# ardaduz/deep-video-mvs

Hardware: AMD Instinct MI355X
Metric: depth frames/sec/GPU @ 320x256x64 planes (fusionnet); rel-L1 vs ref (higher is better)
Workload: dtype f32

## Files before the change

deep-video-mvs_amd/csrc/direct_conv.hip:

```cpp
#include <stdlib.h>

#include "dvmvs_device.h"

namespace dvmvs {

typedef float float4v __attribute__((ext_vector_type(4)));

struct DirectConvArgs {
  const float* x;
  const float* packed;
  const float* bias;
  float* dst;
  float* dst_nhwc;
  long long x_batch_stride, dst_batch_stride;
  int B, C_in, C_out, H, W, OH, OW;
  int act;
  int n_groups;
  int packed_groups;
  int n_chunks;
  int tiles_x;
  int vec4;
};

#ifdef DVMVS_SWEEP_TRACE
constexpr int kDcTraceWords = 8, kDcTraceWaves = 16384;
__device__ unsigned long long g_dc_trace[kDcTraceWaves * kDcTraceWords];
#define DC_TRACE(...) __VA_ARGS__
#define DC_NOW() __builtin_amdgcn_s_memrealtime()
#else
#define DC_TRACE(...)
#endif

constexpr int kDcGroupPad = 16;

__host__ __device__ constexpr int dc_round_to_residue(int v, int mod, int res) { return v + ((res - v) % mod + mod) % mod; }

template <int K_, int S_, int MW_, int MT_, int NT_, int PW_, int KS_, int G_>
struct DirectConvConfig {
  static constexpr int K = K_, S = S_, MW = MW_, MT = MT_, NTILE = NT_, PW = PW_, KS = KS_, G = G_;
  static constexpr int MH = 16 / MW;
  static constexpr int NWAVES = PW * KS, NT = 64 * NWAVES;
  static constexpr int CIC = 4 * KS * G;
  static constexpr int TILE_H = PW * MH, TILE_W = MW * MT;
  static constexpr int PH = (TILE_H - 1) * S + K, PWD = TILE_W * S + 8, PWD4 = PWD / 4;
  static constexpr int SHIFT = 4 - K / 2;
  static constexpr int RS = (MH == 1) ? PWD : dc_round_to_residue(PWD, 16, 8);
  static constexpr int CS = dc_round_to_residue(PH * RS, 64, 16);
  static constexpr int Q = (NTILE * K + 3) / 4;
  static constexpr int NS = G * K;
  static constexpr bool PRIVATE = PW == 1;
  static constexpr int STAGE_CH = PRIVATE ? 4 * G : CIC;
  static constexpr int STAGE_NT = PRIVATE ? 64 : NT;
  static constexpr int PATCH = STAGE_CH * PH * PWD4;
  static constexpr int XREGS = (PATCH + STAGE_NT - 1) / STAGE_NT;
  static constexpr int RED_FLOATS = (KS > 1) ? (KS / 2) * PW * MT * NTILE * 256 : 0;
  static constexpr int BUF = CIC * CS;
  static constexpr bool PREFETCH = XREGS <= 8;
  static constexpr bool DOUBLE = PREFETCH && sizeof(float) * 2 * BUF <= 150 * 1024;
  static constexpr bool WHOLE = DOUBLE && K == 3 && NS * Q <= 6;
  static constexpr int LDS_FLOATS = ((DOUBLE ? 2 : 1) * BUF > RED_FLOATS) ? (DOUBLE ? 2 : 1) * BUF : RED_FLOATS;
  static_assert((MW == 16 || MW == 8) && (TILE_W * S) % 4 == 0 && RS % 4 == 0 && CS % 4 == 0, "tile shape");
  static_assert(NWAVES == 8 && NS >= 2 && (kDcGroupPad % (KS * G)) == 0 && (KS & (KS - 1)) == 0, "workgroup shape");
  static_assert(sizeof(float) * LDS_FLOATS <= 160 * 1024, "LDS");
};

template <class Cfg>
__global__ __launch_bounds__(Cfg::NT) void direct_conv_kernel(DirectConvArgs a) {
  constexpr int K = Cfg::K, S = Cfg::S, MW = Cfg::MW, MT = Cfg::MT, NTILE = Cfg::NTILE, PW = Cfg::PW, KS = Cfg::KS, G = Cfg::G;
  constexpr int MH = Cfg::MH, CIC = Cfg::CIC, PH = Cfg::PH, PWD4 = Cfg::PWD4, RS = Cfg::RS, CS = Cfg::CS, Q = Cfg::Q, NS = Cfg::NS;
  constexpr int XREGS = Cfg::XREGS, PATCH = Cfg::PATCH, STAGE_NT = Cfg::STAGE_NT;
  constexpr bool PRIVATE = Cfg::PRIVATE;
  extern __shared__ __attribute__((aligned(16))) float s_x[];

  const int tid = threadIdx.x, lane = tid & 63, wave = __builtin_amdgcn_readfirstlane(tid >> 6);
  const int pw = wave % PW, ks = wave / PW;
  const int ty = blockIdx.x / a.tiles_x, tx = blockIdx.x - ty * a.tiles_x;
  const int cot = blockIdx.y, b = blockIdx.z;
  const int oy0 = ty * Cfg::TILE_H, ox0 = tx * Cfg::TILE_W;
  const int iy0 = oy0 * S - K / 2, ix0 = ox0 * S - 4;
  const int HW = a.H * a.W;
  DC_TRACE(const unsigned long long tr_start = DC_NOW(); unsigned long long tr_first = 0, tr_req = 0, tr_mfma = 0, tr_store = 0, tr_loop = 0, tr_red = 0, tr_a = 0, tr_b = 0, tr_c = 0;
           auto dump_trace = [&]() __attribute__((always_inline)) {
             const unsigned long long tr_end = DC_NOW();
             const size_t wv = (static_cast<size_t>(blockIdx.z * gridDim.y + blockIdx.y) * gridDim.x + blockIdx.x) * Cfg::NWAVES + (threadIdx.x >> 6);
             if ((threadIdx.x & 63) == 0 && wv < kDcTraceWaves) {
               unsigned long long* t = g_dc_trace + wv * kDcTraceWords;
               t[0] = tr_start; t[1] = tr_first; t[2] = tr_req; t[3] = tr_mfma; t[4] = tr_store; t[5] = tr_loop; t[6] = tr_red; t[7] = tr_end;
             }
           };)
  gcfloat_p xg = as_global(a.x) + static_cast<size_t>(b) * a.x_batch_stride;

  constexpr bool PREFETCH = Cfg::PREFETCH, DOUBLE = Cfg::DOUBLE, WHOLE = Cfg::WHOLE;
  constexpr int BUF = Cfg::BUF;
  const __amdgpu_buffer_rsrc_t x_resource =
      __builtin_amdgcn_make_buffer_rsrc((void*)xg, 0, static_cast<int>(sizeof(float) * static_cast<unsigned int>(a.C_in) * HW), 0x00020000);
  constexpr unsigned int kOutOfRange = 0x80000000u;
  const int stage_tid = PRIVATE ? lane : tid;
  const int stage_ch0 = PRIVATE ? ks * G * 4 : 0;
  auto element_offset = [&](int i) __attribute__((always_inline)) -> unsigned int {
    const int e = stage_tid + i * STAGE_NT;
    const int ch = e / (PH * PWD4), rem = e - ch * (PH * PWD4);
    const int row = rem / PWD4, col4 = rem - row * PWD4;
    const int iy = iy0 + row, ix = ix0 + 4 * col4;
    const bool in = e < PATCH && iy >= 0 && iy < a.H && ix >= 0 && ix < a.W;
    return in ? static_cast<unsigned int>(sizeof(float)) * static_cast<unsigned int>((stage_ch0 + ch) * HW + iy * a.W + ix) : kOutOfRange;
  };
  unsigned int x_offset[PREFETCH ? XREGS : 1];
  if (PREFETCH) {
#pragma unroll
    for (int i = 0; i < XREGS; ++i) x_offset[i] = element_offset(i);
  }
  auto load_element = [&](int chunk, int i) __attribute__((always_inline)) -> float4v {
    const unsigned int offset = PREFETCH ? x_offset[i] : element_offset(i);
    const bool live = chunk * CIC + stage_ch0 + (stage_tid + i * STAGE_NT) / (PH * PWD4) < a.C_in;
    return __builtin_bit_cast(float4v, __builtin_amdgcn_raw_buffer_load_b128(x_resource, static_cast<int>(live ? offset : kOutOfRange),
                                                                             static_cast<int>(sizeof(float) * static_cast<unsigned int>(chunk * CIC) * HW), 0));
  };
  auto store_element = [&](float* buffer, int i, float4v v) __attribute__((always_inline)) {
    const int e = stage_tid + i * STAGE_NT;
    const int ch = e / (PH * PWD4), rem = e - ch * (PH * PWD4);
    const int row = rem / PWD4, col4 = rem - row * PWD4;
    if (e < PATCH) *reinterpret_cast<float4v*>(buffer + (stage_ch0 + ch) * CS + row * RS + 4 * col4) = v;
  };
  float4v xr[PREFETCH ? XREGS : 1];
  auto load_patch = [&](int chunk) __attribute__((always_inline)) {
    if (PREFETCH) {
#pragma unroll
      for (int i = 0; i < XREGS; ++i) xr[i] = load_element(chunk, i);
    }
  };
  auto store_patch = [&](int chunk, float* buffer) __attribute__((always_inline)) {
    if (PREFETCH) {
#pragma unroll
      for (int i = 0; i < XREGS; ++i) store_element(buffer, i, xr[i]);
    } else {
#pragma unroll 1
      for (int i0 = 0; i0 < XREGS; i0 += 4) {
        float4v piece[4];
#pragma unroll
        for (int i = 0; i < 4; ++i) piece[i] = load_element(chunk, i0 + i);
#pragma unroll
        for (int i = 0; i < 4; ++i) store_element(buffer, i0 + i, piece[i]);
      }
    }
  };

  auto chunk_barrier = [&]() __attribute__((always_inline)) {
    if (PRIVATE) __builtin_amdgcn_wave_barrier();
    else __syncthreads();
  };

  const float4v DVMVS_GLOBAL* wq = reinterpret_cast<const float4v DVMVS_GLOBAL*>(as_global(a.packed)) +
                                   static_cast<size_t>(cot) * a.packed_groups * (K * Q * 64) + lane;
  auto load_weights = [&](float4v* w, int cg, int ky) __attribute__((always_inline)) {
    cg = min(cg, a.packed_groups - 1);
#pragma unroll
    for (int q = 0; q < Q; ++q) w[q] = wq[(static_cast<size_t>(cg) * K + ky) * (Q * 64) + q * 64];
  };

  const int m = lane & 15;
  const int a_base = ((lane >> 4) + ks * G * 4) * CS + ((pw * MH + m / MW) * S) * RS + (m % MW) * S + Cfg::SHIFT;

  float4v acc[MT][NTILE];
#pragma unroll
  for (int mt = 0; mt < MT; ++mt)
#pragma unroll
    for (int nt = 0; nt < NTILE; ++nt) acc[mt][nt] = float4v{0.0f, 0.0f, 0.0f, 0.0f};

  auto multiply_step = [&](const float* buffer, int gg, int ky, const float4v* w) __attribute__((always_inline)) {
#pragma unroll
    for (int kx = 0; kx < K; ++kx) {
#pragma unroll
      for (int mt = 0; mt < MT; ++mt) {
        const float av = buffer[a_base + gg * 4 * CS + ky * RS + kx + mt * MW * S];
#pragma unroll
        for (int nt = 0; nt < NTILE; ++nt) {
          const int j = kx * NTILE + nt;
          acc[mt][nt] = __builtin_amdgcn_mfma_f32_16x16x4f32(av, w[j / 4][j % 4], acc[mt][nt], 0, 0, 0);
        }
      }
    }
  };

  if (WHOLE) {
    float4v w_even[NS][Q], w_odd[NS][Q];
    auto whole_chunk = [&](int chunk, float4v(*w_use)[Q], float4v(*w_load)[Q]) __attribute__((always_inline)) {
      const int cg0 = (chunk * KS + ks) * G;
      const float* buffer = s_x + (chunk & 1) * BUF;
      DC_TRACE(tr_a = DC_NOW(); __builtin_amdgcn_sched_barrier(0);)
#pragma unroll
      for (int s = 0; s < NS; ++s) load_weights(w_load[s], ((chunk + 1) * KS + ks) * G + s / K, s % K);
      load_patch(chunk + 1);
      __builtin_amdgcn_sched_barrier(0);
      DC_TRACE(tr_b = DC_NOW(); __builtin_amdgcn_sched_barrier(0);)
#pragma unroll
      for (int s = 0; s < NS; ++s)
        if (cg0 + s / K < a.n_groups) multiply_step(buffer, s / K, s % K, w_use[s]);
      DC_TRACE(__builtin_amdgcn_sched_barrier(0); asm volatile("s_nop 0" ::"v"(acc[0][0]), "v"(acc[MT - 1][NTILE - 1])); tr_c = DC_NOW(); __builtin_amdgcn_sched_barrier(0);)
#pragma unroll
      for (int s = 0; s < NS; ++s) asm volatile("" ::"v"(w_load[s][Q - 1]), "v"(w_use[s][Q - 1]));
      store_patch(chunk + 1, s_x + ((chunk + 1) & 1) * BUF);
      chunk_barrier();
      DC_TRACE(tr_req += tr_b - tr_a; tr_mfma += tr_c - tr_b; tr_store += DC_NOW() - tr_c;)
    };
#pragma unroll
    for (int s = 0; s < NS; ++s) load_weights(w_even[s], ks * G + s / K, s % K);
    load_patch(0);
    store_patch(0, s_x);
    chunk_barrier();
    DC_TRACE(tr_first = DC_NOW();)
    for (int chunk = 0; chunk < a.n_chunks; chunk += 2) {
      whole_chunk(chunk, w_even, w_odd);
      if (chunk + 1 < a.n_chunks) whole_chunk(chunk + 1, w_odd, w_even);
    }
  } else {
    float4v wb[2][Q], w_next[Q];
    load_patch(0);
    load_weights(w_next, ks * G, 0);
    store_patch(0, s_x);
    chunk_barrier();
    DC_TRACE(tr_first = DC_NOW();)
    for (int chunk = 0; chunk < a.n_chunks; ++chunk) {
      const bool more = chunk + 1 < a.n_chunks;
      const int cg0 = (chunk * KS + ks) * G;
      const float* buffer = s_x + (DOUBLE ? (chunk & 1) * BUF : 0);
#pragma unroll
      for (int q = 0; q < Q; ++q) wb[0][q] = w_next[q];
      DC_TRACE(tr_a = tr_b = DC_NOW(); __builtin_amdgcn_sched_barrier(0);)
#pragma unroll
      for (int s = 0; s < NS; ++s) {
        if (s + 1 < NS) load_weights(wb[(s + 1) & 1], cg0 + (s + 1) / K, (s + 1) % K);
        if (s == NS - 2 && (more || DOUBLE)) load_patch(chunk + 1);
        if (s == NS - 1 && (more || DOUBLE)) load_weights(w_next, ((chunk + 1) * KS + ks) * G, 0);
        __builtin_amdgcn_sched_barrier(0);
        if (cg0 + s / K < a.n_groups) multiply_step(buffer, s / K, s % K, wb[s & 1]);
        asm volatile("" ::"v"(wb[s & 1][Q - 1]));
      }
      DC_TRACE(__builtin_amdgcn_sched_barrier(0); asm volatile("s_nop 0" ::"v"(acc[0][0]), "v"(acc[MT - 1][NTILE - 1])); tr_c = DC_NOW(); __builtin_amdgcn_sched_barrier(0);)
      if (DOUBLE) {
        store_patch(chunk + 1, s_x + ((chunk + 1) & 1) * BUF);
        chunk_barrier();
        DC_TRACE(tr_mfma += tr_c - tr_b; tr_store += DC_NOW() - tr_c;)
      } else {
        chunk_barrier();
        if (more) {
          store_patch(chunk + 1, s_x);
          chunk_barrier();
        }
      }
    }
  }

  DC_TRACE(tr_loop = DC_NOW();)
  if (PRIVATE && KS > 1) __syncthreads();
  if (KS > 1) {
    float4v* red = reinterpret_cast<float4v*>(s_x);
#pragma unroll
    for (int half = KS / 2; half >= 1; half >>= 1) {
      if (ks >= half && ks < 2 * half) {
#pragma unroll
        for (int mt = 0; mt < MT; ++mt)
#pragma unroll
          for (int nt = 0; nt < NTILE; ++nt) red[((((ks - half) * PW + pw) * MT + mt) * NTILE + nt) * 64 + lane] = acc[mt][nt];
      }
      __syncthreads();
      if (ks < half) {
#pragma unroll
        for (int mt = 0; mt < MT; ++mt)
#pragma unroll
          for (int nt = 0; nt < NTILE; ++nt) acc[mt][nt] += red[(((ks * PW + pw) * MT + mt) * NTILE + nt) * 64 + lane];
      }
      if (half > 1) __syncthreads();
    }
    if (ks > 0) {
      DC_TRACE(tr_red = DC_NOW(); dump_trace();)
      return;
    }
  }

  const int m0 = (lane >> 4) * 4;
  const int oy = oy0 + pw * MH + m0 / MW;
  DC_TRACE(tr_red = DC_NOW();)
  if (oy >= a.OH) {
    DC_TRACE(dump_trace();)
    return;
  }
  gfloat_p dst = as_global(a.dst) + static_cast<size_t>(b) * a.dst_batch_stride;
#pragma unroll
  for (int nt = 0; nt < NTILE; ++nt) {
    const int co = cot * (16 * NTILE) + nt * 16 + (lane & 15);
    if (co >= a.C_out) continue;
    const float bv = a.bias ? a.bias[co] : 0.0f;
#pragma unroll
    for (int mt = 0; mt < MT; ++mt) {
      const int ox = ox0 + mt * MW + m0 % MW;
      float4v v = acc[mt][nt] + bv;
      if (a.act == 1) {
#pragma unroll
        for (int r = 0; r < 4; ++r) v[r] = fmaxf(v[r], 0.0f);
      }
      gfloat_p d = dst + (static_cast<size_t>(co) * a.OH + oy) * a.OW + ox;
      if (a.vec4 && ox + 3 < a.OW) {
        *reinterpret_cast<float4v DVMVS_GLOBAL*>(d) = v;
      } else {
#pragma unroll
        for (int r = 0; r < 4; ++r)
          if (ox + r < a.OW) d[r] = v[r];
      }
      if (a.dst_nhwc) {
        gfloat_p dn = as_global(a.dst_nhwc) + ((static_cast<size_t>(b) * a.OH + oy) * a.OW + ox) * a.C_out + co;
#pragma unroll
        for (int r = 0; r < 4; ++r)
          if (ox + r < a.OW) dn[static_cast<size_t>(r) * a.C_out] = v[r];
      }
    }
  }
  DC_TRACE(dump_trace();)
}

__global__ __launch_bounds__(256) void direct_conv_pack_kernel(const float* __restrict__ w, float* __restrict__ packed, int C_out, int C_in, int K,
                                                               int n_tile, int packed_groups, long long total) {
  const long long i = static_cast<long long>(blockIdx.x) * 256 + threadIdx.x;
  if (i >= total) return;
  const int Q = (n_tile * K + 3) / 4;
  const int e = static_cast<int>(i & 3), lane = static_cast<int>((i >> 2) & 63);
  long long rest = i >> 8;
  const int q = static_cast<int>(rest % Q);
  rest /= Q;
  const int ky = static_cast<int>(rest % K);
  rest /= K;
  const int cg = static_cast<int>(rest % packed_groups), cot = static_cast<int>(rest / packed_groups);
  const int j = 4 * q + e, kx = j / n_tile, nt = j % n_tile;
  const int co = cot * (16 * n_tile) + nt * 16 + (lane & 15), ci = cg * 4 + (lane >> 4);
  packed[i] = (kx < K && co < C_out && ci < C_in) ? w[((static_cast<size_t>(co) * C_in + ci) * K + ky) * K + kx] : 0.0f;
}

__device__ inline float head_activation(float v, int act, float p0, float p1) {
#pragma clang fp contract(off)
  if (act == 1) return fmaxf(v, 0.0f);
  if (act == 2 || act == 3) {
    const float s = 1.0f / (1.0f + expf(-v));
    return act == 2 ? s : 1.0f / (p0 * s + p1);
  }
  return v;
}

template <int PX>
__global__ __launch_bounds__(256) void conv_head_kernel(const float* __restrict__ x, const float* __restrict__ w, const float* __restrict__ bias,
                                                        float* __restrict__ dst, long long x_batch_stride, long long dst_batch_stride, int C, int H,
                                                        int W, int act, float p0, float p1) {
  constexpr int SL = 256 / PX;
  __shared__ float s_part[SL][PX];
  const int px = threadIdx.x % PX, slice = threadIdx.x / PX;
  const int HW = H * W;
  const int p = blockIdx.x * PX + px, b = blockIdx.y;
  const int y = p / W, xx = p - y * W;
  const int per = (C + SL - 1) / SL;
  const int c_lo = slice * per, c_hi = min(C, c_lo + per);
  float sum = 0.0f;
  if (p < HW) {
    int off[9];
    bool in[9];
#pragma unroll
    for (int t = 0; t < 9; ++t) {
      const int yy = y + t / 3 - 1, xs = xx + t % 3 - 1;
      in[t] = yy >= 0 && yy < H && xs >= 0 && xs < W;
      off[t] = in[t] ? yy * W + xs : 0;
    }
    const float* xb = x + static_cast<size_t>(b) * x_batch_stride;
#pragma unroll 2
    for (int c = c_lo; c < c_hi; ++c) {
      const float* plane = xb + static_cast<size_t>(c) * HW;
      float v[9];
#pragma unroll
      for (int t = 0; t < 9; ++t) v[t] = in[t] ? plane[off[t]] : 0.0f;
#pragma unroll
      for (int t = 0; t < 9; ++t) sum = fmaf(v[t], w[c * 9 + t], sum);
    }
  }
  s_part[slice][px] = sum;
  __syncthreads();
  if (slice == 0 && p < HW) {
    float total = s_part[0][px];
#pragma unroll
    for (int s = 1; s < SL; ++s) total += s_part[s][px];
    if (bias) total += bias[0];
    dst[static_cast<size_t>(b) * dst_batch_stride + p] = head_activation(total, act, p0, p1);
  }
}

struct DirectConvShape {
  int MW, MT, NT, PW, KS;
};
constexpr DirectConvShape kDcShapes[4] = {{16, 5, 2, 4, 2}, {8, 5, 2, 1, 8}, {16, 5, 1, 1, 8}, {8, 5, 1, 1, 8}};
constexpr int kDcCUs = 256;

inline int direct_conv_choose(int B, int C_in, int C_out, int H, int W, int K, int S) {
  if (B <= 0 || C_in <= 0 || C_out <= 0 || C_out % 16 != 0 || (K != 3 && K != 5) || (S != 1 && S != 2) || H <= 0 || W <= 0) return 0;
  if (S == 2 && (H % 2 != 0 || W % 2 != 0)) return 0;
  const int OH = H / S, OW = W / S;
#if defined(DVMVS_SWEEP_TUNING)
  const char* f = getenv("DVMVS_DC_SHAPE");
  const int forced = f ? atoi(f) : 0;
#else
  const int forced = 0;
#endif
  int best = 0;
  double best_fill = 0.0;
  for (int id = 1; id <= 4; ++id) {
    const DirectConvShape& s = kDcShapes[id - 1];
    const int tile_h = s.PW * (16 / s.MW), tile_w = s.MW * s.MT;
    if (OW % tile_w != 0 || C_out % (16 * s.NT) != 0) continue;
    if (forced == id) return id;
    if (forced) continue;
    const long long groups = static_cast<long long>(OW / tile_w) * ((OH + tile_h - 1) / tile_h) * (C_out / (16 * s.NT)) * B;
    const double fill = static_cast<double>(groups) / static_cast<double>(kDcCUs * ((groups + kDcCUs - 1) / kDcCUs));
    if (fill > best_fill + 1e-9) {
      best_fill = fill;
      best = id;
    }
  }
  return best;
}

template <class Cfg>
int launch_direct_conv(DirectConvArgs a, hipStream_t stream) {
  static bool configured[64] = {};
  constexpr size_t lds = sizeof(float) * Cfg::LDS_FLOATS;
  if (lds > 64 * 1024) {
    int device = 0;
    DVMVS_RETURN_IF_HIP(hipGetDevice(&device));
    const bool tracked = device >= 0 && device < 64;
    if (!tracked || !configured[device]) {
      DVMVS_RETURN_IF_HIP(hipFuncSetAttribute(reinterpret_cast<const void*>(direct_conv_kernel<Cfg>), hipFuncAttributeMaxDynamicSharedMemorySize,
                                              static_cast<int>(lds)));
      if (tracked) configured[device] = true;
    }
  }
  a.n_chunks = (a.n_groups + Cfg::KS * Cfg::G - 1) / (Cfg::KS * Cfg::G);
  a.tiles_x = a.OW / Cfg::TILE_W;
  const int tiles_y = (a.OH + Cfg::TILE_H - 1) / Cfg::TILE_H;
  const dim3 grid(a.tiles_x * tiles_y, a.C_out / (16 * Cfg::NTILE), a.B), block(Cfg::NT);
  hipLaunchKernelGGL((direct_conv_kernel<Cfg>), grid, block, lds, stream, a);
  return launch_status();
}

template <int K, int S>
int launch_direct_conv_shape(int id, const DirectConvArgs& a, hipStream_t stream) {
  switch (id) {
    case 1: return launch_direct_conv<DirectConvConfig<K, S, 16, 5, 2, 4, 2, 2>>(a, stream);
    case 2: return launch_direct_conv<DirectConvConfig<K, S, 8, 5, 2, 1, 8, 1>>(a, stream);
    case 3: return launch_direct_conv<DirectConvConfig<K, S, 16, 5, 1, 1, 8, 1>>(a, stream);
    case 4: return launch_direct_conv<DirectConvConfig<K, S, 8, 5, 1, 1, 8, 1>>(a, stream);
  }
  return DVMVS_EUNSUPPORTED;
}

inline int dc_packed_groups(int C_in) { return ((C_in + 3) / 4 + kDcGroupPad - 1) / kDcGroupPad * kDcGroupPad; }

}

extern "C" int dvmvs_direct_conv_tile(int B, int C_in, int H, int W, int C_out, int kernel_size, int stride) {
  const int id = dvmvs::direct_conv_choose(B, C_in, C_out, H, W, kernel_size, stride);
  return id == 0 ? 0 : dvmvs::kDcShapes[id - 1].NT;
}

extern "C" size_t dvmvs_direct_conv_packed_bytes(int C_out, int C_in, int kernel_size, int n_tile) {
  if (C_out <= 0 || C_in <= 0 || (n_tile != 1 && n_tile != 2) || C_out % (16 * n_tile) != 0 || (kernel_size != 3 && kernel_size != 5)) return 0;
  const size_t Q = (n_tile * kernel_size + 3) / 4;
  return sizeof(float) * (C_out / (16 * n_tile)) * dvmvs::dc_packed_groups(C_in) * kernel_size * Q * 256;
}

extern "C" int dvmvs_direct_conv_pack(const float* weight, float* packed, int C_out, int C_in, int kernel_size, int n_tile, dvmvs_stream_t stream) {
  if (!weight || !packed) return DVMVS_EINVAL;
  const size_t bytes = dvmvs_direct_conv_packed_bytes(C_out, C_in, kernel_size, n_tile);
  if (bytes == 0) return DVMVS_EUNSUPPORTED;
  const long long total = static_cast<long long>(bytes / sizeof(float));
  hipLaunchKernelGGL(dvmvs::direct_conv_pack_kernel, dim3(static_cast<unsigned int>((total + 255) / 256)), dim3(256), 0, static_cast<hipStream_t>(stream),
                     weight, packed, C_out, C_in, kernel_size, n_tile, dvmvs::dc_packed_groups(C_in), total);
  return dvmvs::launch_status();
}

extern "C" int dvmvs_direct_conv_fwd(const float* x, long long x_batch_stride, const float* packed, int n_tile, const float* bias, float* dst,
                                     long long dst_batch_stride, int B, int C_in, int H, int W, int C_out, int kernel_size, int stride, int activation,
                                     dvmvs_stream_t stream) {
  return dvmvs_direct_conv_dual_fwd(x, x_batch_stride, packed, n_tile, bias, dst, dst_batch_stride, nullptr, B, C_in, H, W, C_out, kernel_size, stride, activation,
                                    stream);
}

extern "C" int dvmvs_direct_conv_dual_fwd(const float* x, long long x_batch_stride, const float* packed, int n_tile, const float* bias, float* dst,
                                          long long dst_batch_stride, float* dst_nhwc, int B, int C_in, int H, int W, int C_out, int kernel_size, int stride,
                                          int activation, dvmvs_stream_t stream) {
  using namespace dvmvs;
  if (!x || !packed || !dst || B <= 0) return DVMVS_EINVAL;
  if (activation != 0 && activation != 1) return DVMVS_EUNSUPPORTED;
  const int id = direct_conv_choose(B, C_in, C_out, H, W, kernel_size, stride);
  if (id == 0) return DVMVS_EUNSUPPORTED;
  if (kDcShapes[id - 1].NT != n_tile) return DVMVS_EINVAL;
  DirectConvArgs a;
  a.x = x; a.packed = packed; a.bias = bias; a.dst = dst; a.dst_nhwc = dst_nhwc;
  a.B = B; a.C_in = C_in; a.C_out = C_out; a.H = H; a.W = W; a.OH = H / stride; a.OW = W / stride;
  a.x_batch_stride = x_batch_stride ? x_batch_stride : static_cast<long long>(C_in) * H * W;
  a.dst_batch_stride = dst_batch_stride ? dst_batch_stride : static_cast<long long>(C_out) * a.OH * a.OW;
  if (a.x_batch_stride < static_cast<long long>(C_in) * H * W || a.dst_batch_stride < static_cast<long long>(C_out) * a.OH * a.OW) return DVMVS_EINVAL;
  if (W % 4 != 0 || a.x_batch_stride % 4 != 0 || (reinterpret_cast<uintptr_t>(x) & 15) != 0) return DVMVS_EUNSUPPORTED;
  if (static_cast<long long>(C_in + 64) * H * W * 4 >= (1LL << 31)) return DVMVS_EUNSUPPORTED;
  a.act = activation;
  a.n_groups = (C_in + 3) / 4;
  a.packed_groups = dc_packed_groups(C_in);
  a.vec4 = (a.OW % 4 == 0 && (a.OH * a.OW) % 4 == 0 && a.dst_batch_stride % 4 == 0 && (reinterpret_cast<uintptr_t>(dst) & 15) == 0) ? 1 : 0;
  a.n_chunks = 0; a.tiles_x = 0;
  hipStream_t s = static_cast<hipStream_t>(stream);
  if (kernel_size == 3) return stride == 1 ? launch_direct_conv_shape<3, 1>(id, a, s) : launch_direct_conv_shape<3, 2>(id, a, s);
  return stride == 1 ? launch_direct_conv_shape<5, 1>(id, a, s) : launch_direct_conv_shape<5, 2>(id, a, s);
}

extern "C" int dvmvs_conv_head_fwd(const float* x, long long x_batch_stride, const float* weight, const float* bias, float* dst,
                                   long long dst_batch_stride, int B, int C_in, int H, int W, int activation, float p0, float p1, dvmvs_stream_t stream) {
  using namespace dvmvs;
  if (!x || !weight || !dst || B <= 0 || C_in <= 0 || H <= 0 || W <= 0) return DVMVS_EINVAL;
  if (activation < 0 || activation > 3) return DVMVS_EINVAL;
  const long long HW = static_cast<long long>(H) * W;
  if (x_batch_stride == 0) x_batch_stride = HW * C_in;
  if (dst_batch_stride == 0) dst_batch_stride = HW;
  hipStream_t s = static_cast<hipStream_t>(stream);
  if (HW >= 16384) {
    hipLaunchKernelGGL((conv_head_kernel<64>), dim3(static_cast<unsigned int>((HW + 63) / 64), B), dim3(256), 0, s, x, weight, bias, dst, x_batch_stride,
                       dst_batch_stride, C_in, H, W, activation, p0, p1);
  } else {
    hipLaunchKernelGGL((conv_head_kernel<16>), dim3(static_cast<unsigned int>((HW + 15) / 16), B), dim3(256), 0, s, x, weight, bias, dst, x_batch_stride,
                       dst_batch_stride, C_in, H, W, activation, p0, p1);
  }
  return launch_status();
}

#ifdef DVMVS_SWEEP_TRACE
extern "C" int dvmvs_debug_direct_conv_trace(unsigned long long* host, int waves) {
  if (waves > dvmvs::kDcTraceWaves) waves = dvmvs::kDcTraceWaves;
  return static_cast<int>(hipMemcpyFromSymbol(host, HIP_SYMBOL(dvmvs::g_dc_trace), sizeof(unsigned long long) * dvmvs::kDcTraceWords * waves));
}
#endif
```

Measured before the change: 1414.

## Distribute split-K reduction and epilogue across all K-slice waves in direct conv

Replaces the log-tree reduction of split-K partial accumulators, which needed several barrier rounds, with a single LDS dump and one barrier. When KS > 2, each K-slice wave then owns a share of the output tiles, sums all slices for those tiles and writes the epilogue. Before, wave 0 did all the stores. This cuts barriers and spreads the epilogue stores across waves. The cost is a larger LDS reduction buffer (KS instead of KS/2 slices), which may affect the LDS budget and occupancy.

```diff
diff --git a/deep-video-mvs_amd/csrc/direct_conv.hip b/deep-video-mvs_amd/csrc/direct_conv.hip
--- a/deep-video-mvs_amd/csrc/direct_conv.hip
+++ b/deep-video-mvs_amd/csrc/direct_conv.hip
@@ -53,7 +53,7 @@
   static constexpr int STAGE_NT = PRIVATE ? 64 : NT;
   static constexpr int PATCH = STAGE_CH * PH * PWD4;
   static constexpr int XREGS = (PATCH + STAGE_NT - 1) / STAGE_NT;
-  static constexpr int RED_FLOATS = (KS > 1) ? (KS / 2) * PW * MT * NTILE * 256 : 0;
+  static constexpr int RED_FLOATS = (KS > 2) ? KS * PW * MT * NTILE * 256 : (KS / 2) * PW * MT * NTILE * 256;
   static constexpr int BUF = CIC * CS;
   static constexpr bool PREFETCH = XREGS <= 8;
   static constexpr bool DOUBLE = PREFETCH && sizeof(float) * 2 * BUF <= 150 * 1024;
@@ -252,30 +252,47 @@
   }
 
   DC_TRACE(tr_loop = DC_NOW();)
-  if (PRIVATE && KS > 1) __syncthreads();
+  constexpr bool DEAL = KS > 2;
+  constexpr int TILES = MT * NTILE, OWNERS = DEAL ? KS : 1, SHARE = (TILES + OWNERS - 1) / OWNERS;
+  const int t0 = DEAL ? ks * SHARE : 0;
+  float bv[SHARE];
+#pragma unroll
+  for (int i = 0; i < SHARE; ++i) {
+    const int co = cot * (16 * NTILE) + ((t0 + i) / MT) * 16 + (lane & 15);
+    bv[i] = (a.bias && co < a.C_out) ? a.bias[co] : 0.0f;
+  }
+  float4v sum[SHARE];
   if (KS > 1) {
+    if (PRIVATE) __syncthreads();
     float4v* red = reinterpret_cast<float4v*>(s_x);
-#pragma unroll
-    for (int half = KS / 2; half >= 1; half >>= 1) {
-      if (ks >= half && ks < 2 * half) {
-#pragma unroll
-        for (int mt = 0; mt < MT; ++mt)
-#pragma unroll
-          for (int nt = 0; nt < NTILE; ++nt) red[((((ks - half) * PW + pw) * MT + mt) * NTILE + nt) * 64 + lane] = acc[mt][nt];
-      }
-      __syncthreads();
-      if (ks < half) {
-#pragma unroll
-        for (int mt = 0; mt < MT; ++mt)
-#pragma unroll
-          for (int nt = 0; nt < NTILE; ++nt) acc[mt][nt] += red[(((ks * PW + pw) * MT + mt) * NTILE + nt) * 64 + lane];
-      }
-      if (half > 1) __syncthreads();
-    }
-    if (ks > 0) {
+    if (DEAL || ks > 0) {
+#pragma unroll
+      for (int mt = 0; mt < MT; ++mt)
+#pragma unroll
+        for (int nt = 0; nt < NTILE; ++nt) red[(((DEAL ? ks : ks - 1) * PW + pw) * TILES + nt * MT + mt) * 64 + lane] = acc[mt][nt];
+    }
+    __syncthreads();
+    if (!DEAL && ks > 0) {
       DC_TRACE(tr_red = DC_NOW(); dump_trace();)
       return;
     }
+#pragma unroll
+    for (int i = 0; i < SHARE; ++i) {
+      const int t = t0 + i;
+      if (t < TILES) {
+        float4v p[KS];
+#pragma unroll
+        for (int k = 0; k < KS; ++k) p[k] = (DEAL || k > 0) ? red[(((DEAL ? k : k - 1) * PW + pw) * TILES + t) * 64 + lane] : acc[i % MT][i / MT];
+#pragma unroll
+        for (int half = KS / 2; half >= 1; half >>= 1)
+#pragma unroll
+          for (int k = 0; k < half; ++k) p[k] += p[k + half];
+        sum[i] = p[0];
+      }
+    }
+  } else {
+#pragma unroll
+    for (int i = 0; i < SHARE; ++i) sum[i] = acc[i % MT][i / MT];
   }
 
   const int m0 = (lane >> 4) * 4;
@@ -287,32 +304,31 @@
   }
   gfloat_p dst = as_global(a.dst) + static_cast<size_t>(b) * a.dst_batch_stride;
 #pragma unroll
-  for (int nt = 0; nt < NTILE; ++nt) {
+  for (int i = 0; i < SHARE; ++i) {
+    const int t = t0 + i;
+    if (t >= TILES) continue;
+    const int nt = t / MT, mt = t - nt * MT;
     const int co = cot * (16 * NTILE) + nt * 16 + (lane & 15);
     if (co >= a.C_out) continue;
-    const float bv = a.bias ? a.bias[co] : 0.0f;
-#pragma unroll
-    for (int mt = 0; mt < MT; ++mt) {
-      const int ox = ox0 + mt * MW + m0 % MW;
-      float4v v = acc[mt][nt] + bv;
-      if (a.act == 1) {
-#pragma unroll
-        for (int r = 0; r < 4; ++r) v[r] = fmaxf(v[r], 0.0f);
-      }
-      gfloat_p d = dst + (static_cast<size_t>(co) * a.OH + oy) * a.OW + ox;
-      if (a.vec4 && ox + 3 < a.OW) {
-        *reinterpret_cast<float4v DVMVS_GLOBAL*>(d) = v;
-      } else {
-#pragma unroll
-        for (int r = 0; r < 4; ++r)
-          if (ox + r < a.OW) d[r] = v[r];
-      }
-      if (a.dst_nhwc) {
-        gfloat_p dn = as_global(a.dst_nhwc) + ((static_cast<size_t>(b) * a.OH + oy) * a.OW + ox) * a.C_out + co;
-#pragma unroll
-        for (int r = 0; r < 4; ++r)
-          if (ox + r < a.OW) dn[static_cast<size_t>(r) * a.C_out] = v[r];
-      }
+    const int ox = ox0 + mt * MW + m0 % MW;
+    float4v v = sum[i] + bv[i];
+    if (a.act == 1) {
+#pragma unroll
+      for (int r = 0; r < 4; ++r) v[r] = fmaxf(v[r], 0.0f);
+    }
+    gfloat_p d = dst + (static_cast<size_t>(co) * a.OH + oy) * a.OW + ox;
+    if (a.vec4 && ox + 3 < a.OW) {
+      *reinterpret_cast<float4v DVMVS_GLOBAL*>(d) = v;
+    } else {
+#pragma unroll
+      for (int r = 0; r < 4; ++r)
+        if (ox + r < a.OW) d[r] = v[r];
+    }
+    if (a.dst_nhwc) {
+      gfloat_p dn = as_global(a.dst_nhwc) + ((static_cast<size_t>(b) * a.OH + oy) * a.OW + ox) * a.C_out + co;
+#pragma unroll
+      for (int r = 0; r < 4; ++r)
+        if (ox + r < a.OW) dn[static_cast<size_t>(r) * a.C_out] = v[r];
     }
   }
   DC_TRACE(dump_trace();)
```

New measurement: 1435 (median of 6 runs). 1.01x the previous value.
